# Structural-Variant-Calling-with-Pepper/pepper-thesis

Measured on AMD Instinct MI355X. Metric: pileup windows/sec (whole node) + Mbp/sec inferred, HG003 chr20 ONT R9, higher is better.
Workload: dtype f32

## Files before the change

pepper_thesis_amd/csrc/rnn_bf16.hpp:

```cpp
#pragma once
#include "pv_common.hpp"
#include "rnn_plan.hpp"

struct pv_gemm_desc {
    const unsigned char* A;
    const unsigned char* W;
    const float* bias;
    float* C;
    int64_t M;
    int N, K, splits, quads;
    const char* prof_name;
    int terms;
};
int pv_gemm_bf16x3_async(pv_ctx* ctx, const pv_gemm_desc& g, hipStream_t st);
int pv_gemm_bf16x3_prepare();
int pv_upload_split8(const float* w, size_t N, size_t K, unsigned char** d_split, std::vector<void*>& owned);
int pv_upload_split3(const float* w, size_t N, size_t K, unsigned char** d_planes, std::vector<void*>& owned);

struct pv_rec_desc {
    int cell;
    int enc;
    const float* G;
    const unsigned char* wp;
    const unsigned char* wx;
// ... 6 lines not shown
    int T;
    const float* h0;
    float* h_out;
    float* out_f32;
    unsigned char* out_tm;
    unsigned char* out_bm;
    int mt;
    const char* prof_name;
    int tr16;
    const unsigned char* dense_w;
    float* dense_part;
    int x6;
};
int pv_rec_bf16_async(pv_ctx* ctx, const pv_rec_desc& d, hipStream_t st);
int pv_rec_bf16_prepare();
int pv_pack_rec_bf16(const pv_rnn_dir* dirs, int cell, int kx, unsigned char** d_wp, unsigned char** d_wx, std::vector<void*>& owned,
                     int pieces = 2);
int pv_pack_rec_x6(const pv_rnn_dir* dirs, int kx, unsigned char** d_wp, std::vector<void*>& owned);
int pv_pack_gru16_bf16(const pv_rnn_dir* dirs, int kx, unsigned char** d_wp, unsigned char** d_wx, std::vector<void*>& owned);

struct pv_tail_desc {
    const float* part;
    int splits;
    int64_t part_rows;
    const float* b1;
    const unsigned char* wp;
    const float* b[4];
    const float* wo;
    const float* bo;
    float* probs;
    int64_t B;
    unsigned* epoch;
    const int* err;
};
int pv_tail_bf16_async(pv_ctx* ctx, const pv_tail_desc& d, hipStream_t st);
int pv_tail_bf16_prepare();
int pv_pack_tail_bf16(const float* const* w, unsigned char** d_wp, std::vector<void*>& owned);

struct pv_p2_bf16_weights {
    unsigned char* enc_wp = nullptr;
    unsigned char* enc_wx = nullptr;
    unsigned char* dec_wp = nullptr;
    float* enc_bias = nullptr;
    float* enc_bias_hn = nullptr;
    float* dec_bias_hn = nullptr;
    unsigned char* dec_wih_s = nullptr;
    unsigned char* dense_frag = nullptr;
    unsigned char* dense_frag16 = nullptr;
    unsigned char* enc16_wp = nullptr;
    unsigned char* enc16_wx = nullptr;
    unsigned char* dec16_wp = nullptr;
    float* dec_bias_cat = nullptr;
    const float* dense_w = nullptr;
    const float* dense_b = nullptr;
};
int pv_pack_p2_dense(const float* dense_w, unsigned char** d_frag, std::vector<void*>& owned);
int pv_pack_p2_dense16(const float* dense_w, unsigned char** d_frag, std::vector<void*>& owned);
int pv_p2_bf16_forward(pv_ctx* ctx, const pv_p2_plan& pl, const pv_p2_bf16_weights& w, const uint8_t* d_images, int64_t B, uint8_t* d_labels,
                       float* d_acc, hipStream_t st, int seq, int nwin, const float* d_hidden_in, float* d_hidden_out, float* d_logits);
```

pepper_thesis_amd/csrc/rnn_p1.hip:

```cpp
#include "pv_common.hpp"
#include "rnn_bf16.hpp"
#include "rnn_f32.hpp"
#include "rnn_pack_host.hpp"

#include <algorithm>
#include <optional>

namespace {

constexpr int T_STEPS = PV_P1_T;
constexpr int F_IN = PV_P1_F;
constexpr int H = PV_P1_H;
constexpr int ROWS = PV_P1_ROWS;
constexpr int HEAD_N = PV_HEAD_N;
constexpr int HEAD_K = PV_HEAD_K;
constexpr int HEAD_MAX_SPLITS = PV_HEAD_MAX_SPLITS;

}

struct pv_rnn_p1 {
    float* enc_wp[2] = {nullptr, nullptr};
    float* dec_wp[2] = {nullptr, nullptr};
    float* enc_bias = nullptr; float* dec_bias = nullptr;
    float* enc_wps[2] = {nullptr, nullptr};
    float* dec_wps[2] = {nullptr, nullptr};
    void* sp_hx = nullptr; int* sp_flags = nullptr;
    int* sp_err = nullptr;
    unsigned* sp_epoch = nullptr;
    float* w1p = nullptr; float* b1 = nullptr;
    float* wlp[2][4] = {{nullptr, nullptr, nullptr, nullptr}, {nullptr, nullptr, nullptr, nullptr}};
    float* bl[4] = {nullptr, nullptr, nullptr, nullptr};
    float* wo = nullptr; float* bo = nullptr;
    int dtype = PV_DTYPE_F32;
    unsigned char* dec_wih_s = nullptr; float* dec_bias_cat = nullptr;
    unsigned char* w1_s = nullptr;
    unsigned char* enc_rb = nullptr; unsigned char* dec_rb = nullptr;
    unsigned char* tail_wb = nullptr;
    unsigned char* enc_r6 = nullptr; unsigned char* dec_r6 = nullptr;
    unsigned char* dec_wih_p3 = nullptr;
    unsigned char* w1_p3 = nullptr;
    std::vector<void*> owned;
};

static void p1_free(pv_ctx* ctx) {
    if (!ctx->p1) return;
    for (void* p : ctx->p1->owned) (void)hipFree(p);
    delete ctx->p1;
    ctx->p1 = nullptr;
}

void pv_rnn_free(pv_ctx* ctx) {
    p1_free(ctx);
    pv_rnn_free_p2(ctx);
}

extern "C" int pv_rnn_load_p1(pv_ctx* ctx, const pv_weights_p1* w, int dtype) {
    PV_CHECK(ctx && w, PV_ERR_INVALID, "null argument");
    PV_CHECK(dtype == PV_DTYPE_F32 || dtype == PV_DTYPE_BF16_INPUT_GEMM, PV_ERR_INVALID, "unknown dtype %d", dtype);
    for (int d = 0; d < 2; d++) {
        PV_CHECK(w->encoder[d].w_ih && w->encoder[d].w_hh && w->encoder[d].b_ih && w->encoder[d].b_hh &&
                     w->decoder[d].w_ih && w->decoder[d].w_hh && w->decoder[d].b_ih && w->decoder[d].b_hh,
                 PV_ERR_INVALID, "missing LSTM tensor");
    }
    for (int i = 0; i < 5; i++) PV_CHECK(w->linear_w[i] && w->linear_b[i], PV_ERR_INVALID, "missing linear_%d", i + 1);
    PV_CHECK(w->out_w && w->out_b, PV_ERR_INVALID, "missing output layer");
    PV_HIP(hipSetDevice(ctx->device));
    if (ctx->p1) {
        PV_HIP(hipStreamSynchronize(ctx->stream));
        p1_free(ctx);
    }
    pv_rnn_p1* m = new pv_rnn_p1();
    ctx->p1 = m;
    m->dtype = dtype;
// ... 2 lines not shown
    for (int f = 0; f < 2; f++) {
        pack_lstm(w->encoder, F_IN, 32, f ? 16 : 32, wp, bias);
        if ((rc = pv_dev_upload(wp, &m->enc_wp[f], m->owned))) return rc;
        if (!f && (rc = pv_dev_upload(bias, &m->enc_bias, m->owned))) return rc;
        pack_lstm(w->decoder, 2 * H, 2 * H, f ? 16 : 32, wp, bias);
        if ((rc = pv_dev_upload(wp, &m->dec_wp[f], m->owned))) return rc;
        if (!f && (rc = pv_dev_upload(bias, &m->dec_bias, m->owned))) return rc;
    }
    for (int f = 0; f < 2; f++) {
        pack_lstm_split(w->encoder, F_IN, 32, f ? 2 : 4, wp);
        if ((rc = pv_dev_upload(wp, &m->enc_wps[f], m->owned))) return rc;
        pack_lstm_split(w->decoder, 2 * H, 2 * H, f ? 2 : 4, wp);
        if ((rc = pv_dev_upload(wp, &m->dec_wps[f], m->owned))) return rc;
    }
    if ((rc = pv_dev_zeros(PV_LSTM_HX_BYTES, &m->sp_hx, m->owned)) || (rc = pv_dev_zeros(PV_LSTM_FLAGS_BYTES, &m->sp_flags, m->owned)) ||
        (rc = pv_dev_zeros(64, &m->sp_err, m->owned)) || (rc = pv_dev_zeros(64, &m->sp_epoch, m->owned)))
        return rc;
    pack_linear(w->linear_w[0], HEAD_K, 32, wp);
    if ((rc = pv_dev_upload(wp, &m->w1p, m->owned)) || (rc = pv_dev_upload(w->linear_b[0], HEAD_N, &m->b1, m->owned))) return rc;
    for (int i = 0; i < 4; i++) {
        for (int f = 0; f < 2; f++) {
            pack_linear(w->linear_w[i + 1], HEAD_N, f ? 16 : 32, wp);
            if ((rc = pv_dev_upload(wp, &m->wlp[f][i], m->owned))) return rc;
        }
        if ((rc = pv_dev_upload(w->linear_b[i + 1], HEAD_N, &m->bl[i], m->owned))) return rc;
    }
    if ((rc = pv_dev_upload(w->out_w, 3 * HEAD_N, &m->wo, m->owned)) || (rc = pv_dev_upload(w->out_b, 3, &m->bo, m->owned))) return rc;
    std::vector<float> wcat((size_t)2048 * 512), bcat(2048);
    for (int d = 0; d < 2; d++) {
        memcpy(&wcat[(size_t)d * 1024 * 512], w->decoder[d].w_ih, (size_t)1024 * 512 * sizeof(float));
        for (int n = 0; n < 1024; n++) bcat[d * 1024 + n] = w->decoder[d].b_ih[n] + w->decoder[d].b_hh[n];
    }
    if ((rc = pv_dev_upload(bcat, &m->dec_bias_cat, m->owned))) return rc;
    if (dtype == PV_DTYPE_F32) {
        if ((rc = pv_pack_rec_x6(w->encoder, F_IN, &m->enc_r6, m->owned))) return rc;
        if ((rc = pv_pack_rec_x6(w->decoder, 0, &m->dec_r6, m->owned))) return rc;
        if ((rc = pv_upload_split3(wcat.data(), 2048, 512, &m->dec_wih_p3, m->owned))) return rc;
        if ((rc = pv_upload_split3(w->linear_w[0], HEAD_N, HEAD_K, &m->w1_p3, m->owned))) return rc;
        if ((rc = pv_gemm_bf16x3_prepare()) || (rc = pv_rec_bf16_prepare())) return rc;
    }
    if (dtype == PV_DTYPE_BF16_INPUT_GEMM) {
        if ((rc = pv_upload_split8(wcat.data(), 2048, 512, &m->dec_wih_s, m->owned))) return rc;
        if ((rc = pv_upload_split8(w->linear_w[0], HEAD_N, HEAD_K, &m->w1_s, m->owned))) return rc;
        if ((rc = pv_pack_rec_bf16(w->encoder, 4, F_IN, &m->enc_rb, nullptr, m->owned))) return rc;
        if ((rc = pv_pack_rec_bf16(w->decoder, 4, 0, &m->dec_rb, nullptr, m->owned))) return rc;
        const float* tail_w[4] = {w->linear_w[1], w->linear_w[2], w->linear_w[3], w->linear_w[4]};
        if ((rc = pv_pack_tail_bf16(tail_w, &m->tail_wb, m->owned))) return rc;
        if ((rc = pv_gemm_bf16x3_prepare()) || (rc = pv_rec_bf16_prepare()) || (rc = pv_tail_bf16_prepare())) return rc;
    }
    if ((rc = pv_lstm_f32_prepare()) || (rc = pv_head_f32_prepare())) return rc;
    return PV_OK;
}

static int launch_tail(pv_ctx* ctx, const pv_p1_plan& pl, const float* part, int64_t part_rows, float* d_probs, int64_t B, hipStream_t st) {
    const pv_rnn_p1* m = ctx->p1;
    pv_head_tail_desc t = {};
    t.rows = pl.tail_rows; t.part = part; t.b1 = m->b1; t.splits = pl.splits; t.part_rows = part_rows;
    t.wo = m->wo; t.bo = m->bo; t.probs = d_probs; t.B = B; t.epoch = m->sp_epoch; t.err = m->sp_err;
    for (int i = 0; i < 4; i++) { t.wp[i] = m->wlp[pl.tail_rows == 16 ? 1 : 0][i]; t.b[i] = m->bl[i]; }
    int rc = pv_head_tail_async(ctx, t, st);
    if (rc) return rc;
    PV_HIP(hipGetLastError());
    return PV_OK;
}

struct P1Chain {
    int terms;
    const unsigned char *enc_rec, *dec_rec;
    const void *dec_wih, *w1;
    const char* enc_buf;
    const char *n_enc, *n_dec_scope, *n_dec_gemm, *n_dec, *n_lin1;
};

static int p1_forward_mfma(pv_ctx* ctx, const pv_p1_plan& pl, const int8_t* d_images, int64_t B, float* d_probs, float* enc_out,
                           float* dec_out, float* part, hipStream_t st, bool taps) {
    pv_rnn_p1* m = ctx->p1;
    const bool x6 = pl.chain == PV_CHAIN_X6;
    const P1Chain c = x6 ? P1Chain{6, m->enc_r6, m->dec_r6, m->dec_wih_p3, m->w1_p3, "p1.enc_tm", "k_rec_x6_lstm_enc", "k_lstm_layer_dec",
                                   "k_gemm_bf16x6_dec", "k_rec_x6_lstm_dec", "k_gemm_bf16x6_lin1"}
                         : P1Chain{3, m->enc_rb, m->dec_rb, m->dec_wih_s, m->w1_s, "p1.enc_split", "k_rec_bf16_lstm_enc", nullptr,
                                   "k_gemm_bf16x3_dec", "k_rec_bf16_lstm_dec", "k_gemm_bf16x3_lin1"};
    const int64_t Bp = pl.Bp, M = Bp * T_STEPS;
    const size_t out_bytes = (size_t)M * 2 * H * 4;
    unsigned char *enc = nullptr, *dec = reinterpret_cast<unsigned char*>(dec_out);
    float* G = nullptr;
    int rc;
    if ((rc = pv_get(ctx, c.enc_buf, out_bytes, &enc)) || (!x6 && (rc = pv_get(ctx, "p1.dec_split", out_bytes, &dec))) ||
        (rc = pv_get(ctx, "p1.G", (size_t)M * 2048, &G))) return rc;
    pv_rec_desc re = {};
    re.cell = 4; re.enc = 1; re.wp = c.enc_rec; re.bias = m->enc_bias; re.x = d_images; re.x_row_bytes = PV_WINDOW_BYTES; re.x_t0 = 0;
    re.xf = F_IN; re.x_signed = 1; re.B = B; re.Bp = Bp; re.T = T_STEPS; re.out_tm = enc; re.out_f32 = taps ? enc_out : nullptr;
    re.mt = pl.mt; re.x6 = x6; re.prof_name = c.n_enc;
    if ((rc = pv_rec_bf16_async(ctx, re, st))) return rc;
    {
        std::optional<pv_prof_scope> ps;
        if (c.n_dec_scope) ps.emplace(ctx, c.n_dec_scope, st);
        pv_gemm_desc ga = {};
        ga.A = enc; ga.W = static_cast<const unsigned char*>(c.dec_wih); ga.bias = m->dec_bias_cat; ga.C = G; ga.M = M; ga.N = 2048;
        ga.K = 2 * H; ga.splits = 1; ga.quads = 1; ga.terms = c.terms; ga.prof_name = c.n_dec_gemm;
        if ((rc = pv_gemm_bf16x3_async(ctx, ga, st))) return rc;
        pv_rec_desc rd = {};
        rd.cell = 4; rd.enc = 0; rd.G = G; rd.wp = c.dec_rec; rd.B = B; rd.Bp = Bp; rd.T = T_STEPS; rd.out_bm = dec;
        rd.out_f32 = taps && !x6 ? dec_out : nullptr; rd.mt = pl.mt; rd.x6 = x6; rd.prof_name = c.n_dec;
        if ((rc = pv_rec_bf16_async(ctx, rd, st))) return rc;
    }
    pv_gemm_desc gl = {};
    gl.A = dec; gl.W = static_cast<const unsigned char*>(c.w1); gl.bias = nullptr; gl.C = part; gl.M = Bp; gl.N = HEAD_N; gl.K = HEAD_K;
    gl.splits = pl.splits; gl.quads = 0; gl.terms = c.terms; gl.prof_name = c.n_lin1;
    if ((rc = pv_gemm_bf16x3_async(ctx, gl, st))) return rc;
    if (pl.tail == PV_TAIL_HEAD_TAIL) return launch_tail(ctx, pl, part, Bp, d_probs, B, st);
    pv_tail_desc tb = {};
    tb.part = part; tb.b1 = m->b1; tb.splits = pl.splits; tb.part_rows = Bp; tb.wp = m->tail_wb;
    for (int i = 0; i < 4; i++) tb.b[i] = m->bl[i];
    tb.wo = m->wo; tb.bo = m->bo; tb.probs = d_probs; tb.B = B; tb.epoch = m->sp_epoch; tb.err = m->sp_err;
    return pv_tail_bf16_async(ctx, tb, st);
}

static int p1_forward_f32(pv_ctx* ctx, const pv_p1_plan& pl, const int8_t* d_images, int64_t B, float* d_probs, float* enc_out,
                          float* dec_out, float* part, hipStream_t st) {
    pv_rnn_p1* m = ctx->p1;
    const int n_tiles = (int)(pl.Bp / ROWS);
    const bool split = pl.lstm == PV_LSTM_SPLIT4 || pl.lstm == PV_LSTM_SPLIT2;
    const int f = pl.lstm == PV_LSTM_SPLIT4 || pl.lstm == PV_LSTM_ROWS32 ? 0 : 1;
    int rc;
    pv_lstm_desc e = {};
    e.form = pl.lstm;
    e.x_i8 = d_images; e.wp = split ? m->enc_wps[f] : m->enc_wp[f]; e.bias = m->enc_bias; e.out = enc_out; e.B = B; e.n_tiles = n_tiles;
    e.hx = m->sp_hx; e.flags = m->sp_flags; e.epoch = m->sp_epoch; e.err = m->sp_err;
    if ((rc = pv_lstm_f32_async(ctx, e, st))) return rc;
    pv_lstm_desc d = e;
    d.x_i8 = nullptr; d.x_f32 = enc_out; d.wp = split ? m->dec_wps[f] : m->dec_wp[f]; d.bias = m->dec_bias; d.out = dec_out;
    if ((rc = pv_lstm_f32_async(ctx, d, st))) return rc;
    pv_head_splitk_desc h = {};
    h.dec = dec_out; h.w1p = m->w1p; h.part = part; h.B = B; h.n_tiles = n_tiles; h.splits = pl.splits; h.head_map = pl.head_map;
    if ((rc = pv_head_splitk_async(ctx, h, st))) return rc;
    return launch_tail(ctx, pl, part, B, d_probs, B, st);
}

static int p1_forward_launch(pv_ctx* ctx, const int8_t* d_images, int64_t B, float* d_probs, float* enc_out,
                             float* dec_out, float* part, hipStream_t st, bool taps = false) {
    const pv_p1_plan pl = pv_plan_p1(ctx->p1->dtype, B, ctx->num_cu, ctx->opt);
    if (pl.chain != PV_CHAIN_F32) return p1_forward_mfma(ctx, pl, d_images, B, d_probs, enc_out, dec_out, part, st, taps);
    return p1_forward_f32(ctx, pl, d_images, B, d_probs, enc_out, dec_out, part, st);
}

// ... 90 lines not shown
```

pepper_thesis_amd/csrc/rnn_pack_host.hpp:

```cpp
#pragma once
#include <cstddef>
#include <cstdint>
#include <vector>

#include "../../include/pepper_hip.h"
#include "split3_host.hpp"

constexpr int PV_PACK_LSTM_H = 256;
constexpr int PV_PACK_GRU_H = 128;
constexpr int PV_PACK_NCLS = 5;
constexpr int PV_PACK_HEAD_N = 512;

static inline float pack_wval(const pv_rnn_dir& dir, int K, int KP, int HID, int n, int k) {
    if (k < KP) return k < K ? dir.w_ih[(size_t)n * K + k] : 0.0f;
    return dir.w_hh[(size_t)n * HID + (k - KP)];
}

static inline void pack_put_pieces(uint16_t* slot, int lane, int j, float v, int pieces = 2) {
    uint16_t p[3];
    split3_bits(v, p);
    for (int q = 0; q < pieces; q++) slot[512 * q + lane * 8 + j] = p[q];
}

static inline void split8_rows(const float* w, size_t N, size_t K, std::vector<uint16_t>& out) {
// ... 188 lines not shown
    for (int d = 0; d < 2; d++)
        for (int w = 0; w < NW; w++)
            for (int g = 0; g < 3; g++)
                for (int nt = 0; nt < 2; nt++) {
                    auto fill = [&](uint16_t* dst, bool xpart, int ks) {
                        for (int lane = 0; lane < 64; lane++)
                            for (int j = 0; j < 8; j++) {
                                const int n = g * HID + 32 * w + 16 * nt + (lane & 15), k = 32 * ks + 8 * (lane >> 4) + j;
                                const float v = xpart ? (k < kx ? dirs[d].w_ih[(size_t)n * kx + k] : 0.0f) : dirs[d].w_hh[(size_t)n * HID + k];
                                pack_put_pieces(dst, lane, j, v);
                            }
                    };
                    for (int ks = 0; ks < 4; ks++) fill(wp.data() + ((size_t)(d * NW + w) * 24 + (ks * 3 + g) * 2 + nt) * 1024, false, ks);
                    if (kx) fill(wx.data() + ((size_t)(d * NW + w) * 6 + g * 2 + nt) * 1024, true, 0);
                }
}

static inline void pack_tail_bf16(const float* const* w, std::vector<uint16_t>& wp) {
    constexpr int N = PV_PACK_HEAD_N, KS = N / 16;
    wp.assign((size_t)8 * 4 * KS * 2 * 1024, 0);
    for (int wv = 0; wv < 8; wv++)
        for (int l = 0; l < 4; l++)
            for (int ks = 0; ks < KS; ks++)
                for (int g = 0; g < 2; g++) {
                    uint16_t* dst = wp.data() + ((((size_t)wv * 4 + l) * KS + ks) * 2 + g) * 1024;
                    for (int lane = 0; lane < 64; lane++)
                        for (int j = 0; j < 8; j++) {
                            const int n = 64 * wv + 32 * g + (lane & 31), k = 16 * ks + 8 * (lane >> 5) + j;
                            pack_put_pieces(dst, lane, j, w[l][(size_t)n * N + k]);
                        }
                }
}

static inline void pack_p2_dense16(const float* dense_w, std::vector<uint16_t>& f) {
    constexpr int NC = PV_PACK_NCLS, HG = PV_PACK_GRU_H;
    f.assign((size_t)2 * 4 * 1024, 0);
    for (int d = 0; d < 2; d++)
        for (int w = 0; w < 4; w++) {
            uint16_t* dst = f.data() + ((size_t)d * 4 + w) * 1024;
            for (int lane = 0; lane < 64; lane++)
                for (int j = 0; j < 8; j++) {
                    const int n = lane & 15, k = 32 * w + 8 * (lane >> 4) + j;
                    pack_put_pieces(dst, lane, j, n < NC ? dense_w[(size_t)n * 2 * HG + d * HG + k] : 0.0f);
                }
        }
}
static inline void pack_p2_dense(const float* dense_w, std::vector<uint16_t>& f) {
    constexpr int NC = PV_PACK_NCLS, HG = PV_PACK_GRU_H;
    f.assign((size_t)2 * 4 * 2 * 1024, 0);
    for (int d = 0; d < 2; d++)
        for (int w = 0; w < 4; w++)
            for (int kk = 0; kk < 2; kk++) {
                uint16_t* dst = f.data() + (((size_t)d * 4 + w) * 2 + kk) * 1024;
                for (int lane = 0; lane < 64; lane++)
                    for (int j = 0; j < 8; j++) {
                        const int n = lane & 31, k = 16 * (2 * w + kk) + 8 * (lane >> 5) + j;
                        pack_put_pieces(dst, lane, j, n < NC ? dense_w[(size_t)n * 2 * HG + d * HG + k] : 0.0f);
                    }
            }
}
```

pepper_thesis_amd/csrc/rnn_rec_bf16.hip:

```cpp
#include "rnn_bf16.hpp"
#include "mfma_tiles.hpp"
#include "rnn_math.hpp"
#include "rnn_p2_head.hpp"
#include "rnn_pack_host.hpp"

#include <algorithm>
#include <type_traits>
#include <cstdlib>

namespace {

using namespace pvdev;
typedef __bf16 bf16x8 __attribute__((ext_vector_type(8)));
typedef __bf16 bf16x4 __attribute__((ext_vector_type(4)));

__device__ __forceinline__ void split3_rest(float h, __bf16& x1, __bf16& x2) {
#pragma clang fp contract(off)
    const float r1 = h - (float)(__bf16)h;
    x1 = (__bf16)r1;
    x2 = (__bf16)(r1 - (float)x1);
}
__device__ __forceinline__ unsigned split8_off(unsigned k) { return (k >> 3) * 32u + (k & 7u) * 2u; }

#ifdef PV_REC_X6_MFMA32
// ... 116 lines not shown
                    const f32x4 lo = *reinterpret_cast<const f32x4*>(At + m * m_stride + ks * KSB);
                    const f32x4 hi = *reinterpret_cast<const f32x4*>(At + m * m_stride + ks * KSB + 16);
                    ap[1][m] = *reinterpret_cast<const bf16x8*>(At + m * m_stride + ks * KSB + H12);
                    ap[2][m] = *reinterpret_cast<const bf16x8*>(At + m * m_stride + ks * KSB + H12 + 16);
#pragma unroll
                    for (int j = 0; j < 8; j++) ap[0][m][j] = (__bf16)(j < 4 ? lo[j] : hi[j - 4]);
                } else {
                    ap[0][m] = *reinterpret_cast<const bf16x8*>(At + m * m_stride + ks * KSB);
                }
            }
        }
        __builtin_amdgcn_sched_barrier(0);
        {
            const int rs = (I0 + i) % D;
            const bf16x8 b0 = __builtin_bit_cast(bf16x8, bq[rs][0]), b1 = __builtin_bit_cast(bf16x8, bq[rs][1]);
            const bf16x8 b2 = __builtin_bit_cast(bf16x8, bq[rs][2]);
#define PV_X6_TERM(AP, BP)          \
    _Pragma("unroll") for (int m = 0; m < 2; m++) acc[m][g][c] = __builtin_amdgcn_mfma_f32_16x16x32_bf16(ap[AP][m], BP, acc[m][g][c], 0, 0, 0);
            if constexpr (!XP) {
                PV_X6_TERM(2, b0)
                PV_X6_TERM(1, b1)
            }
            PV_X6_TERM(0, b2)
            PV_X6_TERM(0, b0)
            PV_X6_TERM(0, b1)
            if constexpr (!XP) { PV_X6_TERM(1, b0) }
#undef PV_X6_TERM
        }
        hook(i);
        __builtin_amdgcn_sched_barrier(0);
    }
}

#ifndef PV_REC_ABL
#define PV_REC_ABL 0
#endif
#ifdef PV_REC_STAMPS
__device__ unsigned long long g_rec_stamps[8];
#define RSTAMP_REAL(v) asm volatile("s_memrealtime %0\n\ts_waitcnt lgkmcnt(0)" : "=s"(v) :: "memory");
#define RSTAMP(i) { unsigned long long now_; asm volatile("s_memtime %0\n\ts_waitcnt lgkmcnt(0)" : "=s"(now_) :: "memory"); st_acc[i] += now_ - st_last; st_last = now_; }
#else
#define RSTAMP(i)
#endif

template <int NG, bool ENC, int MT, bool X6 = false>
__global__ __launch_bounds__(NG == 4 ? 512 : 256, 1) void k_rec_bf16(RecArgs a) {
    static_assert(!X6 || NG == 4, "split-6 form: LSTM only");
    typedef RecCfg<NG, ENC, MT, X6> C;
    constexpr int NP = X6 ? 3 : 2, SB = NP * 1024;
    constexpr bool M16 = C::M16;
    constexpr int HID = C::HID, NW = C::NW, NTHR = C::NTHR, ROWS = 32 * MT, HS = C::HS, XS = C::XS, D = C::D, NA = C::NA;
    constexpr int NSLOT = C::NSLOT, NXS = C::XRES ? 0 : C::KS_X * NG;
    constexpr int NCOL = 2 * NG * HID;
    extern __shared__ __attribute__((aligned(16))) unsigned char sm[];
    unsigned char* hbuf = sm;
    unsigned char* xbuf = sm + 2 * ROWS * HS;
    const int tid = threadIdx.x, lane = tid & 63, wv = __builtin_amdgcn_readfirstlane(tid >> 6);
    const int xcd = blockIdx.x & 7;
    const int dir = xcd & 1;
    const int tile = (blockIdx.x >> 3) * 4 + (xcd >> 1);
    if (tile >= a.n_tiles) return;
    const int64_t b0 = (int64_t)tile * ROWS;
    const int unit = 32 * wv + (M16 ? (lane & 15) : (lane & 31)), rg = M16 ? lane >> 4 : lane >> 5;
    const int T = a.T;
    const __amdgpu_buffer_rsrc_t wr = make_rsrc(a.wp + (size_t)(dir * NW + wv) * NSLOT * SB);
    const unsigned lane16 = (unsigned)lane * 16u;
    f32x4 bq[C::WRES ? 1 : D][NP];
    bf16x8 wres[C::WRES ? NSLOT : 1][2];
    if constexpr (C::WRES) {
#pragma unroll
        for (int k = 0; k < NSLOT; k++) {
// ... 618 lines not shown
                    *reinterpret_cast<__bf16*>(hn + j * HS + hl[nt] + 16) = lo;
                }
            };
            h_part(0);
            h_part(1);
            if (u == NTL - 1 && s + 1 < T) g_load(tn);
            cell(0);
            cell(1);
        }
        if (s + 1 < T) x_store((s + 1) & 1);
        cur ^= 1;
        lds_barrier();
    }
    tile_out(dir ? 0 : T - 1, cur);
    if (dense) dense_out(dir ? 0 : T - 1, cur);
    if (a.h_out) {
#pragma unroll
        for (int u = 0; u < NTL; u++) {
            if (!live[u]) continue;
#pragma unroll
            for (int nt = 0; nt < 2; nt++)
#pragma unroll
                for (int j = 0; j < 4; j++) a.h_out[((b0[u] + 4 * q + j) * 2 + dir) * HID + 32 * wv + 16 * nt + lr] = st[u][nt][j];
        }
    }
}

template <int NG, bool ENC, int MT, bool X6 = false> constexpr size_t lds_rec() {
    typedef RecCfg<NG, ENC, MT, X6> C;
    return (size_t)2 * 32 * MT * C::HS + (ENC ? (size_t)2 * 32 * MT * C::XS : 0);
}


constexpr int TL_N = PV_HEAD_N, TL_ROWS = PV_TAIL_BF16_ROWS, TL_HS = TL_N * 4 + 16, TL_KS = TL_N / 16, TL_SLOTS = TL_KS * 2, TL_D = 8;
struct TailBfArgs {
    const float* part; int splits; int64_t part_rows;
    const float* b1;
    const unsigned char* wp;
    const float* b[4];
    const float* wo; const float* bo;
    float* probs; int64_t B;
    unsigned* epoch; const int* err;
};
__global__ __launch_bounds__(512, 1) void k_tail_bf16(TailBfArgs a) {
    extern __shared__ __attribute__((aligned(16))) unsigned char sm[];
    unsigned char* tile = sm;
    __shared__ float logits[TL_ROWS][4];
    const int tid = threadIdx.x, lane = tid & 63, wv = __builtin_amdgcn_readfirstlane(tid >> 6), rg = lane >> 5;
    const int64_t b0 = (int64_t)blockIdx.x * TL_ROWS;
    if (a.epoch && blockIdx.x == 0 && tid == 0) atomicAdd(a.epoch, 1u);
    const __amdgpu_buffer_rsrc_t wr = make_rsrc(a.wp + (size_t)wv * 4 * TL_SLOTS * 2048);
    const unsigned lane16 = (unsigned)lane * 16u;
    f32x4 bq[TL_D][2];
#pragma unroll
    for (int k = 0; k < TL_D - 1; k++) {
        bq[k][0] = buf_load4(wr, lane16, (unsigned)(k * 2048));
        bq[k][1] = buf_load4(wr, lane16, (unsigned)(k * 2048 + 1024));
    }
    for (int i = tid; i < TL_ROWS * (TL_N / 4); i += 512) {
        const int row = i / (TL_N / 4), n4 = (i % (TL_N / 4)) * 4;
        int64_t b = b0 + row;
        if (b >= a.B) b = a.B - 1;
        f32x4 v = *reinterpret_cast<const f32x4*>(a.b1 + n4);
        for (int s = 0; s < a.splits; s++) {
            const f32x4 p = *reinterpret_cast<const f32x4*>(a.part + ((size_t)s * a.part_rows + b) * TL_N + n4);
#pragma unroll
            for (int j = 0; j < 4; j++) v[j] += p[j];
        }
        bf16x4 hi, lo;
#pragma unroll
        for (int j = 0; j < 4; j++) {
            const float y = seluf_(v[j]);
            hi[j] = (__bf16)y;
            lo[j] = (__bf16)(y - (float)hi[j]);
        }
        unsigned char* p = tile + row * TL_HS + split8_off((unsigned)n4);
        *reinterpret_cast<bf16x4*>(p) = hi;
        *reinterpret_cast<bf16x4*>(p + 16) = lo;
    }
    __syncthreads();
    const unsigned char* a_h = tile + (lane & 31) * TL_HS + rg * 32;
    auto no_hook = [](int) {};
    auto layer = [&](auto L) {
        constexpr int LI = decltype(L)::value;
        f32x16 acc[2][2];
#pragma unroll
        for (int g = 0; g < 2; g++) {
            const float bv = a.b[LI][64 * wv + 32 * g + (lane & 31)];
#pragma unroll
            for (int m = 0; m < 2; m++)
#pragma unroll
                for (int e = 0; e < 16; e++) acc[m][g][e] = bv;
        }
        ring_bf16<2, 2, 2, TL_D, 4 * TL_SLOTS, LI * TL_SLOTS, TL_KS, false>(acc, a_h, 32 * TL_HS, wr, bq, lane16, no_hook);
        __syncthreads();
#pragma unroll
        for (int m = 0; m < 2; m++)
#pragma unroll
            for (int g = 0; g < 2; g++)
#pragma unroll
                for (int e = 0; e < 16; e++) {
                    const int row = 32 * m + 8 * (e >> 2) + (e & 3) + 4 * rg;
                    const float y = seluf_(acc[m][g][e]);
                    const __bf16 hi = (__bf16)y;
                    const __bf16 lo = (__bf16)(y - (float)hi);
                    unsigned char* p = tile + row * TL_HS + split8_off((unsigned)(64 * wv + 32 * g + (lane & 31)));
                    *reinterpret_cast<__bf16*>(p) = hi;
                    *reinterpret_cast<__bf16*>(p + 16) = lo;
                }
        __syncthreads();
    };
    layer(std::integral_constant<int, 0>());
    layer(std::integral_constant<int, 1>());
    layer(std::integral_constant<int, 2>());
    layer(std::integral_constant<int, 3>());
    {
        const int pair = tid >> 3, sub = tid & 7;
        for (int p = pair; p < TL_ROWS * 3; p += 64) {
            const int row = p / 3, cls = p - row * 3;
            float s = 0.0f;
            for (int k8 = sub; k8 < TL_N / 8; k8 += 8) {
                const bf16x8 hi = *reinterpret_cast<const bf16x8*>(tile + row * TL_HS + k8 * 32);
                const bf16x8 lo = *reinterpret_cast<const bf16x8*>(tile + row * TL_HS + k8 * 32 + 16);
#pragma unroll
                for (int j = 0; j < 8; j++) s += ((float)hi[j] + (float)lo[j]) * a.wo[cls * TL_N + k8 * 8 + j];
            }
            s += __shfl_xor(s, 4, 64);
            s += __shfl_xor(s, 2, 64);
            s += __shfl_xor(s, 1, 64);
            if (sub == 0) logits[row][cls] = s + a.bo[cls];
        }
    }
    __syncthreads();
    if (tid < TL_ROWS) {
        const int64_t b = b0 + tid;
        if (b < a.B) {
            const float l0 = logits[tid][0], l1 = logits[tid][1], l2 = logits[tid][2];
            const float m = fmaxf(l0, fmaxf(l1, l2));
            const float e0 = expf(l0 - m), e1 = expf(l1 - m), e2 = expf(l2 - m);
            const float inv = 1.0f / (e0 + e1 + e2);
            const bool bad = a.err && a.err[0] != 0;
            const float nanv = __builtin_nanf("");
            a.probs[b * 3 + 0] = bad ? nanv : e0 * inv;
            a.probs[b * 3 + 1] = bad ? nanv : e1 * inv;
            a.probs[b * 3 + 2] = bad ? nanv : e2 * inv;
        }
    }
}
constexpr size_t LDS_TAIL_BF = (size_t)TL_ROWS * TL_HS;

}

int pv_pack_rec_bf16(const pv_rnn_dir* dirs, int cell, int kx, unsigned char** d_wp, unsigned char** d_wx, std::vector<void*>& owned,
                     int pieces) {
    PV_CHECK(pieces == 2 || (pieces == 3 && cell == 4), PV_ERR_INVALID, "three-piece fragments exist for the LSTM only");
    std::vector<uint16_t> wp, wx;
    pack_rec_bf16(dirs, cell, kx, pieces, wp, wx);
    if (d_wx) *d_wx = nullptr;
    int rc = pv_dev_upload(wp, d_wp, owned);
    return rc || wx.empty() ? rc : pv_dev_upload(wx, d_wx, owned);
}

int pv_pack_rec_x6(const pv_rnn_dir* dirs, int kx, unsigned char** d_wp, std::vector<void*>& owned) {
    std::vector<uint16_t> wp, wx;
    if (REC_X6_16) pack_rec_x6_16(dirs, kx, wp);
    else pack_rec_bf16(dirs, 4, kx, 3, wp, wx);
    return pv_dev_upload(wp, d_wp, owned);
}

int pv_pack_gru16_bf16(const pv_rnn_dir* dirs, int kx, unsigned char** d_wp, unsigned char** d_wx, std::vector<void*>& owned) {
    std::vector<uint16_t> wp, wx;
    pack_gru16_bf16(dirs, kx, wp, wx);
    if (d_wx) *d_wx = nullptr;
    int rc = pv_dev_upload(wp, d_wp, owned);
    return rc || wx.empty() ? rc : pv_dev_upload(wx, d_wx, owned);
}

int pv_pack_tail_bf16(const float* const* w, unsigned char** d_wp, std::vector<void*>& owned) {
    static_assert(TL_N == PV_PACK_HEAD_N, "pack_tail_bf16 packs 512 x 512 layers");
    std::vector<uint16_t> wp;
    pack_tail_bf16(w, wp);
    return pv_dev_upload(wp, d_wp, owned);
}

int pv_tail_bf16_prepare() {
    PV_HIP(hipFuncSetAttribute((const void*)k_tail_bf16, hipFuncAttributeMaxDynamicSharedMemorySize, (int)LDS_TAIL_BF));
    return PV_OK;
}

int pv_tail_bf16_async(pv_ctx* ctx, const pv_tail_desc& d, hipStream_t st) {
    PV_CHECK(d.part && d.wp && d.probs && d.B > 0 && d.splits >= 1, PV_ERR_INVALID, "bad tail launch");
    TailBfArgs a;
    a.part = d.part; a.splits = d.splits; a.part_rows = d.part_rows; a.b1 = d.b1; a.wp = d.wp;
    for (int i = 0; i < 4; i++) a.b[i] = d.b[i];
    a.wo = d.wo; a.bo = d.bo; a.probs = d.probs; a.B = d.B; a.epoch = d.epoch; a.err = d.err;
    pv_prof_scope ps(ctx, "k_tail_bf16", st);
    k_tail_bf16<<<(unsigned)((d.B + TL_ROWS - 1) / TL_ROWS), 512, LDS_TAIL_BF, st>>>(a);
    PV_HIP(hipGetLastError());
    return PV_OK;
}

int pv_rec_bf16_prepare() {
#define PV_REC_ATTR(NG, ENC, MT) \
    PV_HIP(hipFuncSetAttribute((const void*)k_rec_bf16<NG, ENC, MT>, hipFuncAttributeMaxDynamicSharedMemorySize, (int)lds_rec<NG, ENC, MT>()))
    PV_REC_ATTR(4, true, 1); PV_REC_ATTR(4, true, 2); PV_REC_ATTR(4, false, 1); PV_REC_ATTR(4, false, 2);
    PV_REC_ATTR(3, true, 1); PV_REC_ATTR(3, true, 2); PV_REC_ATTR(3, false, 1); PV_REC_ATTR(3, false, 2);
#undef PV_REC_ATTR
#define PV_REC_ATTR6(ENC, MT) \
    PV_HIP(hipFuncSetAttribute((const void*)k_rec_bf16<4, ENC, MT, true>, hipFuncAttributeMaxDynamicSharedMemorySize, (int)lds_rec<4, ENC, MT, true>()))
    PV_REC_ATTR6(true, 1); PV_REC_ATTR6(false, 1);
#undef PV_REC_ATTR6
    return PV_OK;
}

int pv_rec_bf16_async(pv_ctx* ctx, const pv_rec_desc& d, hipStream_t st) {
    PV_CHECK((d.cell == 3 || d.cell == 4) && d.T > 0 && (d.tr16 || ((d.mt == 1 || d.mt == 2) && d.Bp % (32 * d.mt) == 0)), PV_ERR_INVALID, "bad recurrent-layer launch");
    PV_CHECK(!d.x6 || (d.cell == 4 && !d.tr16 && d.mt == 1), PV_ERR_INVALID, "the split-6 form is an LSTM layer on 32-row tiles");
    RecArgs a;
    a.G = d.G; a.wp = d.wp; a.wx = d.wx; a.bias = d.bias; a.bias_hn = d.bias_hn; a.x = (const unsigned char*)d.x;
    a.x_row_bytes = d.x_row_bytes; a.x_t0 = d.x_t0; a.xf = d.xf; a.x_signed = d.x_signed; a.B = d.B; a.Bp = d.Bp; a.T = d.T;
    a.h0 = d.h0; a.h_out = d.h_out; a.out_f32 = d.out_f32; a.out_tm = d.out_tm; a.out_bm = d.out_bm;
    a.n_tiles = d.tr16 ? 0 : (int)(d.Bp / (32 * d.mt));
    a.dw = d.dense_w; a.dpart = d.dense_part;
    PV_CHECK(!d.dense_part || (d.cell == 3 && !d.enc && d.dense_w), PV_ERR_INVALID, "the dense layer folds into the GRU decoder only");
    if (d.tr16) {
        PV_CHECK(d.cell == 3 && (d.tr16 == 1 || d.tr16 == 2) && d.Bp % 16 == 0 && !d.out_f32 && !(d.dense_part && d.enc), PV_ERR_INVALID, "bad 16-row GRU launch");
        a.n_tiles = (int)(d.Bp / 16);
        const int ntl = d.tr16;
        const int n_wg = (a.n_tiles + ntl - 1) / ntl;
        const unsigned grid16 = (unsigned)(((n_wg + 3) / 4) * 8);
// ... 153 lines not shown
        d.cell = 3; d.enc = 0; d.G = G; d.wp = w.dec_wp; d.bias_hn = w.dec_bias_hn; d.B = B; d.Bp = Bp; d.T = p2::WIN;
        d.h0 = state; d.h_out = state; d.mt = mt; d.prof_name = "k_rec_bf16_gru_dec";
        if (tr16) { d.tr16 = tr16; d.wp = w.dec16_wp; d.prof_name = "k_gru16_bf16_dec"; }
        float* lg_out = (d_logits && wi == nwin - 1) ? d_logits : nullptr;
        if (fold_dense) {
            d.dense_w = tr16 ? w.dense_frag16 : w.dense_frag; d.dense_part = dpart;
            if ((rc = pv_rec_bf16_async(ctx, d, st))) return rc;
            pv_prof_scope ps(ctx, "k_p2_combine", st);
            const int64_t nthr = (int64_t)p2::WIN * B;
            if (tr16) k_p2_combine<16><<<(unsigned)((nthr + 255) / 256), 256, 0, st>>>(dpart, Bp, B, w.dense_b, d_acc, seq, ws, lg_out);
            else k_p2_combine<32><<<(unsigned)((nthr + 255) / 256), 256, 0, st>>>(dpart, Bp, B, w.dense_b, d_acc, seq, ws, lg_out);
        } else {
            d.out_tm = dec;
            if ((rc = pv_rec_bf16_async(ctx, d, st))) return rc;
            pv_prof_scope ps(ctx, "k_p2_dense", st);
            const int64_t nthr = (int64_t)p2::WIN * B * 8;
            k_p2_dense<<<(unsigned)((nthr + 255) / 256), 256, 0, st>>>(dec, Bp, B, w.dense_w, w.dense_b, d_acc, seq, ws, lg_out);
        }
    }
    if (d_hidden_out) k_p2_state_out<<<(unsigned)((B * 2 * p2::HG + 255) / 256), 256, 0, st>>>(state, d_hidden_out, B);
    if (d_labels) k_p2_argmax<<<(unsigned)((B * seq + 255) / 256), 256, 0, st>>>(d_acc, B * seq, d_labels);
    PV_HIP(hipGetLastError());
    return PV_OK;
}

#ifdef PV_REC_STAMPS
extern "C" int pv_debug_rec_stamps(unsigned long long* out5) {
    unsigned long long z[8] = {0, 0, 0, 0, 0, 0, 0, 0};
    PV_HIP(hipDeviceSynchronize());
    PV_HIP(hipMemcpyFromSymbol(out5, HIP_SYMBOL(g_rec_stamps), 5 * sizeof(unsigned long long)));
    PV_HIP(hipMemcpyToSymbol(HIP_SYMBOL(g_rec_stamps), z, sizeof z));
    return PV_OK;
}
extern "C" int pv_debug_rec_clock(unsigned long long* out2) {
    PV_HIP(hipDeviceSynchronize());
    PV_HIP(hipMemcpyFromSymbol(out2, HIP_SYMBOL(g_rec_stamps), 2 * sizeof(unsigned long long), 5 * sizeof(unsigned long long)));
    return PV_OK;
}
#endif
```

Measured before the change: 1.146 million.

## Add fused bf16x3 MFMA head tail kernel for the f32 x6 path

Adds a three-piece (bf16x3, six-term) variant of the fused head-tail kernel, packing the four 512x512 tail layers into three bf16 planes. It runs on the f32 path when x6 is set and tail_rows is 32, replacing the previous launch_tail path. The goal is to emulate f32 accuracy using MFMA bf16 with a deep weight-prefetch ring and the activation tile kept in LDS. The cost is a larger LDS tile holding an f32 copy plus two residual planes, and six MFMAs per k-step instead of fewer.

```diff
diff --git a/pepper_thesis_amd/csrc/rnn_bf16.hpp b/pepper_thesis_amd/csrc/rnn_bf16.hpp
--- a/pepper_thesis_amd/csrc/rnn_bf16.hpp
+++ b/pepper_thesis_amd/csrc/rnn_bf16.hpp
@@ -62,10 +62,11 @@
     int64_t B;
     unsigned* epoch;
     const int* err;
+    int x6;
 };
 int pv_tail_bf16_async(pv_ctx* ctx, const pv_tail_desc& d, hipStream_t st);
 int pv_tail_bf16_prepare();
-int pv_pack_tail_bf16(const float* const* w, unsigned char** d_wp, std::vector<void*>& owned);
+int pv_pack_tail_bf16(const float* const* w, unsigned char** d_wp, std::vector<void*>& owned, int pieces = 2);
 
 struct pv_p2_bf16_weights {
     unsigned char* enc_wp = nullptr;
diff --git a/pepper_thesis_amd/csrc/rnn_p1.hip b/pepper_thesis_amd/csrc/rnn_p1.hip
--- a/pepper_thesis_amd/csrc/rnn_p1.hip
+++ b/pepper_thesis_amd/csrc/rnn_p1.hip
@@ -39,6 +39,7 @@
     unsigned char* enc_r6 = nullptr; unsigned char* dec_r6 = nullptr;
     unsigned char* dec_wih_p3 = nullptr;
     unsigned char* w1_p3 = nullptr;
+    unsigned char* tail_w6 = nullptr;
     std::vector<void*> owned;
 };
 
@@ -107,19 +108,20 @@
         for (int n = 0; n < 1024; n++) bcat[d * 1024 + n] = w->decoder[d].b_ih[n] + w->decoder[d].b_hh[n];
     }
     if ((rc = pv_dev_upload(bcat, &m->dec_bias_cat, m->owned))) return rc;
+    const float* tail_w[4] = {w->linear_w[1], w->linear_w[2], w->linear_w[3], w->linear_w[4]};
     if (dtype == PV_DTYPE_F32) {
         if ((rc = pv_pack_rec_x6(w->encoder, F_IN, &m->enc_r6, m->owned))) return rc;
         if ((rc = pv_pack_rec_x6(w->decoder, 0, &m->dec_r6, m->owned))) return rc;
         if ((rc = pv_upload_split3(wcat.data(), 2048, 512, &m->dec_wih_p3, m->owned))) return rc;
         if ((rc = pv_upload_split3(w->linear_w[0], HEAD_N, HEAD_K, &m->w1_p3, m->owned))) return rc;
-        if ((rc = pv_gemm_bf16x3_prepare()) || (rc = pv_rec_bf16_prepare())) return rc;
+        if ((rc = pv_pack_tail_bf16(tail_w, &m->tail_w6, m->owned, 3))) return rc;
+        if ((rc = pv_gemm_bf16x3_prepare()) || (rc = pv_rec_bf16_prepare()) || (rc = pv_tail_bf16_prepare())) return rc;
     }
     if (dtype == PV_DTYPE_BF16_INPUT_GEMM) {
         if ((rc = pv_upload_split8(wcat.data(), 2048, 512, &m->dec_wih_s, m->owned))) return rc;
         if ((rc = pv_upload_split8(w->linear_w[0], HEAD_N, HEAD_K, &m->w1_s, m->owned))) return rc;
         if ((rc = pv_pack_rec_bf16(w->encoder, 4, F_IN, &m->enc_rb, nullptr, m->owned))) return rc;
         if ((rc = pv_pack_rec_bf16(w->decoder, 4, 0, &m->dec_rb, nullptr, m->owned))) return rc;
-        const float* tail_w[4] = {w->linear_w[1], w->linear_w[2], w->linear_w[3], w->linear_w[4]};
         if ((rc = pv_pack_tail_bf16(tail_w, &m->tail_wb, m->owned))) return rc;
         if ((rc = pv_gemm_bf16x3_prepare()) || (rc = pv_rec_bf16_prepare()) || (rc = pv_tail_bf16_prepare())) return rc;
     }
@@ -183,9 +185,10 @@
     gl.A = dec; gl.W = static_cast<const unsigned char*>(c.w1); gl.bias = nullptr; gl.C = part; gl.M = Bp; gl.N = HEAD_N; gl.K = HEAD_K;
     gl.splits = pl.splits; gl.quads = 0; gl.terms = c.terms; gl.prof_name = c.n_lin1;
     if ((rc = pv_gemm_bf16x3_async(ctx, gl, st))) return rc;
-    if (pl.tail == PV_TAIL_HEAD_TAIL) return launch_tail(ctx, pl, part, Bp, d_probs, B, st);
+    const bool tail6 = x6 && pl.tail == PV_TAIL_HEAD_TAIL && pl.tail_rows == 32;
+    if (pl.tail == PV_TAIL_HEAD_TAIL && !tail6) return launch_tail(ctx, pl, part, Bp, d_probs, B, st);
     pv_tail_desc tb = {};
-    tb.part = part; tb.b1 = m->b1; tb.splits = pl.splits; tb.part_rows = Bp; tb.wp = m->tail_wb;
+    tb.part = part; tb.b1 = m->b1; tb.splits = pl.splits; tb.part_rows = Bp; tb.wp = tail6 ? m->tail_w6 : m->tail_wb; tb.x6 = tail6;
     for (int i = 0; i < 4; i++) tb.b[i] = m->bl[i];
     tb.wo = m->wo; tb.bo = m->bo; tb.probs = d_probs; tb.B = B; tb.epoch = m->sp_epoch; tb.err = m->sp_err;
     return pv_tail_bf16_async(ctx, tb, st);
diff --git a/pepper_thesis_amd/csrc/rnn_pack_host.hpp b/pepper_thesis_amd/csrc/rnn_pack_host.hpp
--- a/pepper_thesis_amd/csrc/rnn_pack_host.hpp
+++ b/pepper_thesis_amd/csrc/rnn_pack_host.hpp
@@ -244,6 +244,23 @@
                 }
 }
 
+static inline void pack_tail_x6(const float* const* w, std::vector<uint16_t>& wp) {
+    constexpr int N = PV_PACK_HEAD_N, KS = N / 16;
+    constexpr size_t SL = 3 * 512;
+    wp.assign((size_t)8 * 4 * KS * 2 * SL, 0);
+    for (int wv = 0; wv < 8; wv++)
+        for (int l = 0; l < 4; l++)
+            for (int ks = 0; ks < KS; ks++)
+                for (int g = 0; g < 2; g++) {
+                    uint16_t* dst = wp.data() + ((((size_t)wv * 4 + l) * KS + ks) * 2 + g) * SL;
+                    for (int lane = 0; lane < 64; lane++)
+                        for (int j = 0; j < 8; j++) {
+                            const int n = 64 * wv + 32 * g + (lane & 31), k = 16 * ks + 8 * (lane >> 5) + j;
+                            pack_put_pieces(dst, lane, j, w[l][(size_t)n * N + k], 3);
+                        }
+                }
+}
+
 static inline void pack_p2_dense16(const float* dense_w, std::vector<uint16_t>& f) {
     constexpr int NC = PV_PACK_NCLS, HG = PV_PACK_GRU_H;
     f.assign((size_t)2 * 4 * 1024, 0);
diff --git a/pepper_thesis_amd/csrc/rnn_rec_bf16.hip b/pepper_thesis_amd/csrc/rnn_rec_bf16.hip
--- a/pepper_thesis_amd/csrc/rnn_rec_bf16.hip
+++ b/pepper_thesis_amd/csrc/rnn_rec_bf16.hip
@@ -172,11 +172,56 @@
     }
 }
 
+template <int DK, int NKTOT, int K0, int NKS, int H12>
+__device__ __forceinline__ void ring_tail_x6(f32x16 (&acc)[1][2], const unsigned char* __restrict__ At, __amdgpu_buffer_rsrc_t wr,
+                                             f32x4 (&bq)[DK][2][3], unsigned lane16) {
+    f32x4 raw[2];
+    bf16x8 ap[3], nx[2];
+    auto a_load = [&](int ks) {
+        raw[0] = *reinterpret_cast<const f32x4*>(At + ks * 64);
+        raw[1] = *reinterpret_cast<const f32x4*>(At + ks * 64 + 16);
+        nx[0] = *reinterpret_cast<const bf16x8*>(At + ks * 64 + H12);
+        nx[1] = *reinterpret_cast<const bf16x8*>(At + ks * 64 + H12 + 16);
+    };
+    a_load(0);
+#pragma unroll
+    for (int ks = 0; ks < NKS; ks++) {
+        {
+            const int kv = (K0 + ks + DK - 1) % NKTOT, rs = (K0 + ks + DK - 1) % DK;
+#pragma unroll
+            for (int g = 0; g < 2; g++)
+#pragma unroll
+                for (int p = 0; p < 3; p++) bq[rs][g][p] = buf_load4(wr, lane16, (unsigned)((kv * 2 + g) * 3072 + p * 1024));
+        }
+#pragma unroll
+        for (int j = 0; j < 8; j++) ap[0][j] = (__bf16)(j < 4 ? raw[0][j] : raw[1][j - 4]);
+        ap[1] = nx[0];
+        ap[2] = nx[1];
+        if (ks + 1 < NKS) a_load(ks + 1);
+        __builtin_amdgcn_sched_barrier(0);
+        {
+            const int rs = (K0 + ks) % DK;
+#define PV_T6_TERM(AP, BP)          \
+    _Pragma("unroll") for (int g = 0; g < 2; g++)             \
+        acc[0][g] = __builtin_amdgcn_mfma_f32_32x32x16_bf16(ap[AP], __builtin_bit_cast(bf16x8, bq[rs][g][BP]), acc[0][g], 0, 0, 0);
+            PV_T6_TERM(2, 0)
+            PV_T6_TERM(1, 1)
+            PV_T6_TERM(0, 2)
+            PV_T6_TERM(0, 0)
+            PV_T6_TERM(0, 1)
+            PV_T6_TERM(1, 0)
+#undef PV_T6_TERM
+        }
+        __builtin_amdgcn_sched_barrier(0);
+    }
+}
+
 #ifndef PV_REC_ABL
 #define PV_REC_ABL 0
 #endif
 #ifdef PV_REC_STAMPS
 __device__ unsigned long long g_rec_stamps[8];
+__device__ unsigned long long g_tail_stamps[5];
 #define RSTAMP_REAL(v) asm volatile("s_memrealtime %0\n\ts_waitcnt lgkmcnt(0)" : "=s"(v) :: "memory");
 #define RSTAMP(i) { unsigned long long now_; asm volatile("s_memtime %0\n\ts_waitcnt lgkmcnt(0)" : "=s"(now_) :: "memory"); st_acc[i] += now_ - st_last; st_last = now_; }
 #else
@@ -861,7 +906,13 @@
 }
 
 
-constexpr int TL_N = PV_HEAD_N, TL_ROWS = PV_TAIL_BF16_ROWS, TL_HS = TL_N * 4 + 16, TL_KS = TL_N / 16, TL_SLOTS = TL_KS * 2, TL_D = 8;
+constexpr int TL_N = PV_HEAD_N, TL_KS = TL_N / 16, TL_SLOTS = TL_KS * 2, TL_D = 8, TL_DK = 5;
+template <bool X6> struct TailCfg {
+    static constexpr int ROWS = X6 ? PV_P1_ROWS : PV_TAIL_BF16_ROWS, MT = ROWS / 32;
+    static constexpr int HS = TL_N * (X6 ? 8 : 4) + 16, H12 = X6 ? TL_N * 4 : 0;
+    static constexpr int NP = X6 ? 3 : 2, SB = NP * 1024;
+    static constexpr size_t LDS = (size_t)ROWS * HS;
+};
 struct TailBfArgs {
     const float* part; int splits; int64_t part_rows;
     const float* b1;
@@ -871,73 +922,126 @@
     float* probs; int64_t B;
     unsigned* epoch; const int* err;
 };
+template <bool X6>
 __global__ __launch_bounds__(512, 1) void k_tail_bf16(TailBfArgs a) {
+    typedef TailCfg<X6> C;
+    constexpr int TL_ROWS = C::ROWS, TL_HS = C::HS, MT = C::MT, NP = C::NP, SB = C::SB;
     extern __shared__ __attribute__((aligned(16))) unsigned char sm[];
     unsigned char* tile = sm;
     __shared__ float logits[TL_ROWS][4];
     const int tid = threadIdx.x, lane = tid & 63, wv = __builtin_amdgcn_readfirstlane(tid >> 6), rg = lane >> 5;
     const int64_t b0 = (int64_t)blockIdx.x * TL_ROWS;
     if (a.epoch && blockIdx.x == 0 && tid == 0) atomicAdd(a.epoch, 1u);
-    const __amdgpu_buffer_rsrc_t wr = make_rsrc(a.wp + (size_t)wv * 4 * TL_SLOTS * 2048);
+    const __amdgpu_buffer_rsrc_t wr = make_rsrc(a.wp + (size_t)wv * 4 * TL_SLOTS * SB);
     const unsigned lane16 = (unsigned)lane * 16u;
-    f32x4 bq[TL_D][2];
-#pragma unroll
-    for (int k = 0; k < TL_D - 1; k++) {
-        bq[k][0] = buf_load4(wr, lane16, (unsigned)(k * 2048));
-        bq[k][1] = buf_load4(wr, lane16, (unsigned)(k * 2048 + 1024));
-    }
+    f32x4 bq[X6 ? 1 : TL_D][NP];
+    f32x4 bk[X6 ? TL_DK : 1][2][3];
+    if constexpr (X6) {
+#pragma unroll
+        for (int k = 0; k < TL_DK - 1; k++)
+#pragma unroll
+            for (int g = 0; g < 2; g++)
+#pragma unroll
+                for (int p = 0; p < 3; p++) bk[k][g][p] = buf_load4(wr, lane16, (unsigned)((k * 2 + g) * SB + p * 1024));
+    } else {
+#pragma unroll
+        for (int k = 0; k < TL_D - 1; k++)
+#pragma unroll
+            for (int p = 0; p < NP; p++) bq[k][p] = buf_load4(wr, lane16, (unsigned)(k * SB + p * 1024));
+    }
+#ifdef PV_REC_STAMPS
+    unsigned long long st_acc[5] = {0, 0, 0, 0, 0}, st_last;
+    asm volatile("s_memtime %0\n\ts_waitcnt lgkmcnt(0)" : "=s"(st_last) :: "memory");
+#endif
     for (int i = tid; i < TL_ROWS * (TL_N / 4); i += 512) {
         const int row = i / (TL_N / 4), n4 = (i % (TL_N / 4)) * 4;
         int64_t b = b0 + row;
         if (b >= a.B) b = a.B - 1;
         f32x4 v = *reinterpret_cast<const f32x4*>(a.b1 + n4);
-        for (int s = 0; s < a.splits; s++) {
-            const f32x4 p = *reinterpret_cast<const f32x4*>(a.part + ((size_t)s * a.part_rows + b) * TL_N + n4);
-#pragma unroll
-            for (int j = 0; j < 4; j++) v[j] += p[j];
-        }
-        bf16x4 hi, lo;
-#pragma unroll
-        for (int j = 0; j < 4; j++) {
-            const float y = seluf_(v[j]);
-            hi[j] = (__bf16)y;
-            lo[j] = (__bf16)(y - (float)hi[j]);
-        }
-        unsigned char* p = tile + row * TL_HS + split8_off((unsigned)n4);
-        *reinterpret_cast<bf16x4*>(p) = hi;
-        *reinterpret_cast<bf16x4*>(p + 16) = lo;
+        if constexpr (X6) {
+#pragma unroll 11
+            for (int s = 0; s < a.splits; s++) {
+                const f32x4 p = *reinterpret_cast<const f32x4*>(a.part + ((size_t)s * a.part_rows + b) * TL_N + n4);
+#pragma unroll
+                for (int j = 0; j < 4; j++) v[j] += p[j];
+            }
+            f32x4 y;
+            bf16x4 x1, x2;
+#pragma unroll
+            for (int j = 0; j < 4; j++) {
+                y[j] = seluf_(v[j]);
+                __bf16 p1, p2;
+                split3_rest(y[j], p1, p2);
+                x1[j] = p1; x2[j] = p2;
+            }
+            *reinterpret_cast<f32x4*>(tile + row * TL_HS + n4 * 4) = y;
+            unsigned char* p = tile + row * TL_HS + C::H12 + split8_off((unsigned)n4);
+            *reinterpret_cast<bf16x4*>(p) = x1;
+            *reinterpret_cast<bf16x4*>(p + 16) = x2;
+        } else {
+            for (int s = 0; s < a.splits; s++) {
+                const f32x4 p = *reinterpret_cast<const f32x4*>(a.part + ((size_t)s * a.part_rows + b) * TL_N + n4);
+#pragma unroll
+                for (int j = 0; j < 4; j++) v[j] += p[j];
+            }
+            bf16x4 hi, lo;
+#pragma unroll
+            for (int j = 0; j < 4; j++) {
+                const float y = seluf_(v[j]);
+                hi[j] = (__bf16)y;
+                lo[j] = (__bf16)(y - (float)hi[j]);
+            }
+            unsigned char* p = tile + row * TL_HS + split8_off((unsigned)n4);
+            *reinterpret_cast<bf16x4*>(p) = hi;
+            *reinterpret_cast<bf16x4*>(p + 16) = lo;
+        }
     }
     __syncthreads();
+    RSTAMP(0)
     const unsigned char* a_h = tile + (lane & 31) * TL_HS + rg * 32;
     auto no_hook = [](int) {};
     auto layer = [&](auto L) {
         constexpr int LI = decltype(L)::value;
-        f32x16 acc[2][2];
+        f32x16 acc[MT][2];
 #pragma unroll
         for (int g = 0; g < 2; g++) {
             const float bv = a.b[LI][64 * wv + 32 * g + (lane & 31)];
 #pragma unroll
-            for (int m = 0; m < 2; m++)
+            for (int m = 0; m < MT; m++)
 #pragma unroll
                 for (int e = 0; e < 16; e++) acc[m][g][e] = bv;
         }
-        ring_bf16<2, 2, 2, TL_D, 4 * TL_SLOTS, LI * TL_SLOTS, TL_KS, false>(acc, a_h, 32 * TL_HS, wr, bq, lane16, no_hook);
+        if constexpr (X6) ring_tail_x6<TL_DK, 4 * TL_KS, LI * TL_KS, TL_KS, C::H12>(acc, a_h, wr, bk, lane16);
+        else ring_bf16<2, MT, 2, TL_D, 4 * TL_SLOTS, LI * TL_SLOTS, TL_KS, false>(acc, a_h, 32 * TL_HS, wr, bq, lane16, no_hook);
+        RSTAMP(1)
         __syncthreads();
-#pragma unroll
-        for (int m = 0; m < 2; m++)
+        RSTAMP(2)
+#pragma unroll
+        for (int m = 0; m < MT; m++)
 #pragma unroll
             for (int g = 0; g < 2; g++)
 #pragma unroll
                 for (int e = 0; e < 16; e++) {
                     const int row = 32 * m + 8 * (e >> 2) + (e & 3) + 4 * rg;
+                    const unsigned col = (unsigned)(64 * wv + 32 * g + (lane & 31));
                     const float y = seluf_(acc[m][g][e]);
-                    const __bf16 hi = (__bf16)y;
-                    const __bf16 lo = (__bf16)(y - (float)hi);
-                    unsigned char* p = tile + row * TL_HS + split8_off((unsigned)(64 * wv + 32 * g + (lane & 31)));
-                    *reinterpret_cast<__bf16*>(p) = hi;
-                    *reinterpret_cast<__bf16*>(p + 16) = lo;
+                    if constexpr (X6) {
+                        *reinterpret_cast<float*>(tile + row * TL_HS + col * 4u) = y;
+                        __bf16 p1, p2;
+                        split3_rest(y, p1, p2);
+                        unsigned char* p = tile + row * TL_HS + C::H12 + split8_off(col);
+                        *reinterpret_cast<__bf16*>(p) = p1;
+                        *reinterpret_cast<__bf16*>(p + 16) = p2;
+                    } else {
+                        const __bf16 hi = (__bf16)y;
+                        const __bf16 lo = (__bf16)(y - (float)hi);
+                        unsigned char* p = tile + row * TL_HS + split8_off(col);
+                        *reinterpret_cast<__bf16*>(p) = hi;
+                        *reinterpret_cast<__bf16*>(p + 16) = lo;
+                    }
                 }
         __syncthreads();
+        RSTAMP(3)
     };
     layer(std::integral_constant<int, 0>());
     layer(std::integral_constant<int, 1>());
@@ -948,11 +1052,20 @@
         for (int p = pair; p < TL_ROWS * 3; p += 64) {
             const int row = p / 3, cls = p - row * 3;
             float s = 0.0f;
-            for (int k8 = sub; k8 < TL_N / 8; k8 += 8) {
-                const bf16x8 hi = *reinterpret_cast<const bf16x8*>(tile + row * TL_HS + k8 * 32);
-                const bf16x8 lo = *reinterpret_cast<const bf16x8*>(tile + row * TL_HS + k8 * 32 + 16);
-#pragma unroll
-                for (int j = 0; j < 8; j++) s += ((float)hi[j] + (float)lo[j]) * a.wo[cls * TL_N + k8 * 8 + j];
+            if constexpr (X6) {
+                const float* src = reinterpret_cast<const float*>(tile + row * TL_HS);
+                float wk[TL_N / 8];
+#pragma unroll
+                for (int i = 0; i < TL_N / 8; i++) wk[i] = a.wo[cls * TL_N + sub + 8 * i];
+#pragma unroll
+                for (int i = 0; i < TL_N / 8; i++) s = __builtin_fmaf(src[sub + 8 * i], wk[i], s);
+            } else {
+                for (int k8 = sub; k8 < TL_N / 8; k8 += 8) {
+                    const bf16x8 hi = *reinterpret_cast<const bf16x8*>(tile + row * TL_HS + k8 * 32);
+                    const bf16x8 lo = *reinterpret_cast<const bf16x8*>(tile + row * TL_HS + k8 * 32 + 16);
+#pragma unroll
+                    for (int j = 0; j < 8; j++) s += ((float)hi[j] + (float)lo[j]) * a.wo[cls * TL_N + k8 * 8 + j];
+                }
             }
             s += __shfl_xor(s, 4, 64);
             s += __shfl_xor(s, 2, 64);
@@ -975,8 +1088,12 @@
             a.probs[b * 3 + 2] = bad ? nanv : e2 * inv;
         }
     }
-}
-constexpr size_t LDS_TAIL_BF = (size_t)TL_ROWS * TL_HS;
+#ifdef PV_REC_STAMPS
+    RSTAMP(4)
+    if (blockIdx.x == 0 && lane == 0)
+        for (int i = 0; i < 5; i++) atomicAdd(&g_tail_stamps[i], st_acc[i]);
+#endif
+}
 
 }
 
@@ -1005,15 +1122,18 @@
     return rc || wx.empty() ? rc : pv_dev_upload(wx, d_wx, owned);
 }
 
-int pv_pack_tail_bf16(const float* const* w, unsigned char** d_wp, std::vector<void*>& owned) {
+int pv_pack_tail_bf16(const float* const* w, unsigned char** d_wp, std::vector<void*>& owned, int pieces) {
     static_assert(TL_N == PV_PACK_HEAD_N, "pack_tail_bf16 packs 512 x 512 layers");
+    PV_CHECK(pieces == 2 || pieces == 3, PV_ERR_INVALID, "two or three pieces");
     std::vector<uint16_t> wp;
-    pack_tail_bf16(w, wp);
+    if (pieces == 3) pack_tail_x6(w, wp);
+    else pack_tail_bf16(w, wp);
     return pv_dev_upload(wp, d_wp, owned);
 }
 
 int pv_tail_bf16_prepare() {
-    PV_HIP(hipFuncSetAttribute((const void*)k_tail_bf16, hipFuncAttributeMaxDynamicSharedMemorySize, (int)LDS_TAIL_BF));
+    PV_HIP(hipFuncSetAttribute((const void*)k_tail_bf16<false>, hipFuncAttributeMaxDynamicSharedMemorySize, (int)TailCfg<false>::LDS));
+    PV_HIP(hipFuncSetAttribute((const void*)k_tail_bf16<true>, hipFuncAttributeMaxDynamicSharedMemorySize, (int)TailCfg<true>::LDS));
     return PV_OK;
 }
 
@@ -1023,8 +1143,9 @@
     a.part = d.part; a.splits = d.splits; a.part_rows = d.part_rows; a.b1 = d.b1; a.wp = d.wp;
     for (int i = 0; i < 4; i++) a.b[i] = d.b[i];
     a.wo = d.wo; a.bo = d.bo; a.probs = d.probs; a.B = d.B; a.epoch = d.epoch; a.err = d.err;
-    pv_prof_scope ps(ctx, "k_tail_bf16", st);
-    k_tail_bf16<<<(unsigned)((d.B + TL_ROWS - 1) / TL_ROWS), 512, LDS_TAIL_BF, st>>>(a);
+    pv_prof_scope ps(ctx, d.x6 ? "k_head_tail" : "k_tail_bf16", st);
+    if (d.x6) k_tail_bf16<true><<<(unsigned)((d.B + TailCfg<true>::ROWS - 1) / TailCfg<true>::ROWS), 512, TailCfg<true>::LDS, st>>>(a);
+    else k_tail_bf16<false><<<(unsigned)((d.B + TailCfg<false>::ROWS - 1) / TailCfg<false>::ROWS), 512, TailCfg<false>::LDS, st>>>(a);
     PV_HIP(hipGetLastError());
     return PV_OK;
 }
@@ -1244,6 +1365,13 @@
     PV_HIP(hipMemcpyToSymbol(HIP_SYMBOL(g_rec_stamps), z, sizeof z));
     return PV_OK;
 }
+extern "C" int pv_debug_tail_stamps(unsigned long long* out5) {
+    unsigned long long z[5] = {0, 0, 0, 0, 0};
+    PV_HIP(hipDeviceSynchronize());
+    PV_HIP(hipMemcpyFromSymbol(out5, HIP_SYMBOL(g_tail_stamps), sizeof z));
+    PV_HIP(hipMemcpyToSymbol(HIP_SYMBOL(g_tail_stamps), z, sizeof z));
+    return PV_OK;
+}
 extern "C" int pv_debug_rec_clock(unsigned long long* out2) {
     PV_HIP(hipDeviceSynchronize());
     PV_HIP(hipMemcpyFromSymbol(out2, HIP_SYMBOL(g_rec_stamps), 2 * sizeof(unsigned long long), 5 * sizeof(unsigned long long)));
```

Measured after the change: 1.166 million (median of 6 runs). 1.02x the previous value.
